# vishal-2000/EDMP

Hardware: AMD Instinct MI355X
Metric: guided denoise-steps/sec (trajectories x reverse steps) (higher is better)
Workload: dtype f32

## Files before the change

### edmp_amd/_capi.py

```python
from __future__ import annotations

import ctypes as C
import os

_HERE = os.path.dirname(os.path.abspath(__file__))
LIB_PATH = os.path.join(_HERE, "libedmp_hip.so")

MAX_LEVELS = 8
MAX_SCENES = 16
MAX_OBSTACLES = 64
MAX_SPHERES = 128
MAX_SWEEP_SUBSTEPS = 64
MAX_REPAIR_ITERS = 1024


class UNetDesc(C.Structure):
    _fields_ = [
        ("input_dim", C.c_int32),
        ("time_dim", C.c_int32),
        ("n_levels", C.c_int32),
        ("dims", C.c_int32 * MAX_LEVELS),
        ("horizon", C.c_int32),
        ("T", C.c_int32),
    ]
# ... 77 lines not shown
    "edmp_unet_flops_direct": (_i, [_vp, _pd]),
    "edmp_unet_flops_pipes": (_i, [_vp, _pd, _pd]),
    "edmp_prof_ops_bf16": (_i, [_vp, _i, C.POINTER(C.c_int), _pd]),
    "edmp_unet_slot": (_i, [_vp, C.c_uint64]),
    "edmp_guide_slot": (_i, [_vp, C.c_uint64]),
    "edmp_argmin_dev": (_i, [_vp, _vp, _i, C.POINTER(C.c_int)]),
    "edmp_sdf_set": (_i, [_vp, _pf, _i, _pi32, _pd, _pd, _i, _i]),
    "edmp_sdf_set_self": (_i, [_vp, _pi32, _pd, _pd, _i, _i]),
    "edmp_sdf_self_rows_dev": (_i, [_vp, _vp, _i, _i, _i, _i, _i, _vp, _vp]),
    "edmp_sdf_set_goal": (_i, [_vp, _pd, _pd, _pi32, _pd, _pd, _i]),
    "edmp_sdf_goal_rows_dev": (_i, [_vp, _vp, _i, _i, _i, _i, _i, _vp, _vp, _vp, _vp]),
    "edmp_sdf_set_sweep": (_i, [_vp, _pd, _pi32, _i]),
    "edmp_sdf_sweep_rows_dev": (_i, [_vp, _vp, _i, _i, _i, _pd, _pd, _i, _vp, _vp]),
    "edmp_scenes_sdf_sweep_rows_dev": (_i, [_vp, _vp, _i, _i, _i, _i, _pd, _pd, _i, _vp, _vp]),
    "edmp_sdf_repair_rows_dev": (_i, [_vp, _vp, _i, _i, _pd, _pd, _pi32, _i, _i, _i, _d, _d, _d, _d, _vp, _vp, _vp]),
    "edmp_scenes_sdf_repair_rows_dev": (_i, [_vp, _vp, _i, _i, _i, _pd, _pd, _pi32, _i, _i, _i, _d, _d, _d, _d, _vp, _vp, _vp]),
    "edmp_sdf_rows_dev": (_i, [_vp, _vp, _i, _i, _i, _pd, _pd, _vp, _vp]),
    "edmp_scene_batch_set_sdf": (_i, [_vp, _pf, _i, _pi32, _pd, _pd, _i, _i, _i]),
    "edmp_scenes_sdf_rows_dev": (_i, [_vp, _vp, _i, _i, _i, _i, _pd, _pd, _vp, _vp]),
    "edmp_sampler_set_allreduce": (_i, [_vp, _vp, _vp]),
    "edmp_rccl_load": (_i, [C.c_char_p]),
    "edmp_rccl_unique_id": (_i, [_vp]),
    "edmp_rccl_attach": (_i, [_vp, _vp, _i, _i]),
    "edmp_rccl_attach_comm": (_i, [_vp, _vp]),
    "edmp_rccl_enable": (_i, [_vp, _i]),
    "edmp_rccl_detach": (_i, [_vp]),
    "edmp_rccl_info": (_i, [_vp, _pi32]),
    "edmp_sampler_allreduce_stats": (_i, [_vp, C.POINTER(C.c_uint64), _i]),
    "edmp_prof_enable": (_i, [_vp, _i]),
    "edmp_prof_read": (_i, [_vp, _pd, C.POINTER(C.c_int64), _i]),
    "edmp_prof_ops": (_i, [_vp, _i, C.POINTER(C.c_int), _pd, C.POINTER(C.c_int64), _pd, C.c_char_p]),
    "edmp_unet_op_attrs": (_i, [_vp, _i, C.POINTER(C.c_int), C.c_char_p, _pi32, _pi32, _pi32, _pi32]),
    "edmp_cu_claim": (_i, [_i, _i, _i, _i]),
}

_lib = None


def load():
    global _lib
    if _lib is not None:
        return _lib
    if not os.path.exists(LIB_PATH):
        raise EdmpError(
            f"{LIB_PATH} is missing: build it with `python -c 'import __graft_entry__ as g; g.build()'` "
            "(hipcc --offload-arch=gfx950).  edmp_amd has no CPU fallback."
        )
    try:
        import torch
    except ImportError:
        pass
    try:
        lib = C.CDLL(LIB_PATH)
    except OSError as e:
        raise EdmpError(f"cannot load {LIB_PATH}: {e}") from e
    for name, (res, args) in SIGNATURES.items():
        try:
            fn = getattr(lib, name)
        except AttributeError as e:
            raise EdmpError(f"{LIB_PATH} does not export {name}") from e
        fn.restype = res
        fn.argtypes = args
    _lib = lib
    return lib


def check(rc: int, what: str = ""):
    if rc != 0:
        msg = load().edmp_last_error()
        err = (EdmpLayoutError if rc == ERR_LAYOUT else EdmpError)(f"{what or 'libedmp_hip'} failed (rc={rc}): {msg.decode() if msg else '?'}")
        err.rc = rc
        raise err


def as_pd(a):
    return a.ctypes.data_as(_pd)


def as_pf(a):
    return a.ctypes.data_as(_pf)


def as_pi32(a):
    return a.ctypes.data_as(_pi32)


def plan_describe(input_dim, time_dim, dims, horizon, T):
    lib = load()
    d = UNetDesc()
    d.input_dim, d.time_dim, d.n_levels, d.horizon, d.T = input_dim, time_dim, len(dims), horizon, T
    for i, v in enumerate(dims):
        d.dims[i] = v
    n, layout, size = C.c_int(), C.c_int(), C.c_int64()
    check(lib.edmp_unet_plan_describe(C.byref(d), 0, C.byref(n), None, None, None), "edmp_unet_plan_describe")
    names = C.create_string_buffer(max(n.value, 1) * 64)
    check(lib.edmp_unet_plan_describe(C.byref(d), n.value, C.byref(n), names, C.byref(layout), C.byref(size)), "edmp_unet_plan_describe")
    return [names.raw[i * 64:(i + 1) * 64].split(b"\0", 1)[0].decode() for i in range(n.value)], layout.value, size.value
```

### edmp_amd/csrc/bf3.hip

```cpp
#pragma once
#include <type_traits>

#include "params.h"
#include "wide.hip"

namespace edmp {

constexpr int kBf3Threads = 512;

typedef __attribute__((ext_vector_type(8))) __bf16 bf16x8_t;
typedef __attribute__((ext_vector_type(2))) __bf16 bf16x2_t;
typedef __attribute__((ext_vector_type(4))) float f32x4_t;
typedef __attribute__((ext_vector_type(4))) unsigned u32x4_t;
typedef __attribute__((ext_vector_type(2))) unsigned u32x2_t;

inline unsigned short bf16_rne_bits(float x) {
    unsigned u = __builtin_bit_cast(unsigned, x);
    u += 0x7fffu + ((u >> 16) & 1u);
    return (unsigned short)(u >> 16);
}
inline float bf16_bits_to_float(unsigned short b) { return __builtin_bit_cast(float, (unsigned)b << 16); }
inline void split3_bf16_rne(float x, unsigned short (&c)[3]) {
    c[0] = bf16_rne_bits(x);
    const float r1 = x - bf16_bits_to_float(c[0]);
    c[1] = bf16_rne_bits(r1);
    const float r2 = r1 - bf16_bits_to_float(c[1]);
    c[2] = bf16_rne_bits(r2);
}

template <int KIND, int MS, int CG, int GS, int LIN, bool RES>
struct Bf3Cfg {
    static constexpr int kKind = KIND, kMs = MS, kCg = CG, kGs = GS, kLin = LIN;
    static constexpr bool kRes = RES;
    static constexpr int NTH = kBf3Threads, NMW = 4;
    static constexpr int LOUT = (KIND == WK_K5) ? LIN : (KIND == WK_DOWN) ? (LIN - 1) / 2 + 1 : ((2 * LIN == 8 || 2 * LIN == 14 || 2 * LIN == 26) ? 2 * LIN - 1 : 2 * LIN);
    static constexpr bool GN = (KIND == WK_K5);
    static constexpr bool PAIRABLE = !GN && MS == 32 && CG == 32;
    using Paired = std::conditional_t<PAIRABLE, Bf3Cfg<KIND, MS, 2 * CG, 2 * CG, LIN, RES>, Bf3Cfg>;
    static constexpr int SW = 16, S = CG / SW, PARTS = NMW / S;
    static constexpr bool ROWSPLIT = (PARTS == 2 && MS == 32);
    static constexpr int NR = (PARTS == 1) ? MS / 16 : 1;
    static constexpr bool RES_ONE_ACC = RES && MS == 16 && LIN >= 13;
    static constexpr int KC = 32;
    static constexpr int RS = KC + 8;
    static constexpr int PLANE = MS * RS;
    static constexpr int STAGE = LIN * 3 * PLANE;
    static constexpr int NTAP = (KIND == WK_K5) ? 5 : (KIND == WK_DOWN) ? 3 : 4;
    static constexpr int NSLOT = NTAP + (RES ? 1 : 0);
    static constexpr int WBLK = NSLOT * 3 * 1024;
    static constexpr int slot(int l, int lp) {
        const int t = (KIND == WK_K5) ? lp - l + 2 : (KIND == WK_DOWN) ? lp - 2 * l + 1 : l + 1 - 2 * lp;
        return (t >= 0 && t < NTAP) ? t : -1;
    }
    static constexpr int NTILE = LOUT + (RES ? LIN : 0);
    static constexpr int tslot(int tile, int lp) { return tile < LOUT ? slot(tile, lp) : (tile - LOUT == lp ? NTAP : -1); }
    static constexpr int pairs_of(int l) {
        int n = (RES && l < LIN) ? 1 : 0;
        for (int lp = 0; lp < LIN; ++lp) n += slot(l, lp) >= 0 ? 1 : 0;
        return n;
    }
    static constexpr int total_pairs() {
        int n = 0;
        for (int l = 0; l < LOUT; ++l) n += pairs_of(l);
        return n;
    }
    static constexpr unsigned part0_mask() {
        if (ROWSPLIT || PARTS == 1) return ~0u;
        const int tot = total_pairs();
        int pc[16] = {};
        for (int l = 0; l < LOUT; ++l) pc[l] = pairs_of(l);
        unsigned best = 0;
// ... 5 lines not shown
            if (mx < bestmax) bestmax = mx, best = m;
        }
        return best;
    }
    static constexpr unsigned P0 = part0_mask();
    static constexpr bool owned(int tile, int H) {
        if (ROWSPLIT || PARTS == 1) return true;
        const int l = tile < LOUT ? tile : tile - LOUT;
        return (int)((P0 >> l) & 1u) == (H == 0 ? 1 : 0);
    }
    static constexpr int local(int tile, int H) {
        int n = 0;
        for (int q = 0; q < tile; ++q) n += owned(q, H) ? 1 : 0;
        return n;
    }
    static constexpr int ntiles(int H) { return local(NTILE, H); }
    static constexpr int MAXT = ntiles(0) > ntiles(1) ? ntiles(0) : ntiles(1);
    static constexpr bool needed(int H, int lp) {
        for (int t = 0; t < NTILE; ++t)
            if (owned(t, H) && tslot(t, lp) >= 0) return true;
        return false;
    }
    static constexpr int ord(int H, int q) {
        int n = 0;
        for (int i = 0; i < q; ++i) n += needed(H, i % LIN) ? 1 : 0;
        return n;
    }
    static constexpr int next(int H, int q) {
        for (int i = q + 1; i < 2 * LIN; ++i)
            if (needed(H, i % LIN)) return i;
        return -1;
    }
    static constexpr int first(int H) { return needed(H, 0) ? 0 : next(H, 0); }
    static constexpr bool DEALT = !(KIND == WK_DOWN && MS == 32);
    static constexpr int DEAL = 1;
    static constexpr int nfeed(int H, int lp, int upto = NTILE) {
        int n = 0;
        for (int t = 0; t < upto; ++t) n += (owned(t, H) && tslot(t, lp) >= 0) ? 1 : 0;
        return n;
    }
    static constexpr int nslots(int H, int q) { return DEALT ? 3 * nfeed(H, q % LIN) * NR / DEAL : 0; }
    static constexpr int nreads(int H, int q) {
        const int qn = next(H, q);
        return qn < 0 ? 0 : NR * (qn / LIN == 0 ? 2 : 3);
    }
    static constexpr int reads_dealt(int H, int q) {
        const int qn = next(H, q);
        if (qn < 0 || (ROTATE && next(H, qn) < 0)) return 0;
        return nreads(H, q) < nslots(H, q) ? nreads(H, q) : nslots(H, q);
    }
    static constexpr int nweights(int ph) { return !DEALT ? 0 : ph == 0 ? NSLOT : 2 * NSLOT; }
    static constexpr int wbase(int H, int ph, int lp) {
        int n = 0;
        for (int i = 0; i < lp; ++i)
            if (needed(H, i)) {
                const int cap = nslots(H, ph * LIN + i) - reads_dealt(H, ph * LIN + i);
                n += cap < nweights(ph) - n ? cap : nweights(ph) - n;
            }
        return n;
    }
    static constexpr int wdealt(int H, int q) { return wbase(H, q / LIN, q % LIN + 1) - wbase(H, q / LIN, q % LIN); }
    static constexpr int KREGS = MAXT * NR * 8 + 3 * NSLOT * 4 + 2 * NR * 3 * 4;
    static constexpr bool ROTATE = KREGS <= 240, BIAS_EARLY = ROTATE;
    static_assert(DEALT || ROTATE, "the burst form of the K loop is kept for rotated instances only");
    static constexpr int A_F4 = LIN * MS * (KC / 4);
    static constexpr int NA = (A_F4 + 255) / 256;
    static constexpr int YS = LOUT * CG + 4, RYS = LIN * CG + 4;
    static constexpr int PPR = NTH / MS, ROW_F4 = LOUT * CG / 4, NF4 = (ROW_F4 + PPR - 1) / PPR;
    static constexpr int RROW_F4 = LIN * CG / 4, RNF4 = (RROW_F4 + PPR - 1) / PPR;
    static constexpr size_t lds_bytes() {
        const size_t a = 2 * (size_t)STAGE * 2, y = (size_t)MS * (YS + (RES ? RYS : 0)) * 4;
        return a > y ? a : y;
    }
    static_assert((CG == 32 && S == 2 && PARTS == 2) || (CG == 64 && S == 4 && PARTS == 1 && MS == 32), "two 16-channel slabs x two parts, or four slabs = the four MFMA waves");
    static_assert(MS == 32 || MS == 16, "32 samples (sample-half parts) or 16 samples (position-set parts)");
    static_assert(!RES || KIND == WK_K5, "the folded residual 1x1 conv belongs to a Conv1dBlock");
    static_assert(!GN || CG % GS == 0, "whole GroupNorm groups per workgroup");
    static_assert((4 * PPR) % CG == 0, "a thread's columns of the final pass lie in one GroupNorm group");
    static_assert(LOUT <= 16, "part0_mask searches 2^LOUT subsets");
};

#ifdef EDMP_BF3_STAMPS
__device__ long long g_bf3_stamps[8][8];
#define EDMP_BF3_STAMP(i) \
    if (blockIdx.x == 0 && lane == 0) g_bf3_stamps[wave][i] = clock64();
#define EDMP_BF3_CHUNK_BARRIER \
    bar_t0 = clock64();        \
    __syncthreads();           \
    bar_t1 = clock64();
#define EDMP_BF3_BAR_ADD bar_cyc += bar_t1 - bar_t0;
#else
#define EDMP_BF3_STAMP(i)
#define EDMP_BF3_CHUNK_BARRIER __syncthreads();
#define EDMP_BF3_BAR_ADD
#endif

template <class Cf, class Claim>
__device__ __forceinline__ void bf3_conv_body(const float* a_src1, const float* a_src2, const void* a_W, int a_C1, int a_C2, int a_Cout, int a_B, int a_gx_shift, int a_ng_shift, const RcbP& p, Claim claim) {
    constexpr int KIND = Cf::kKind, MS = Cf::kMs, CG = Cf::kCg, GS = Cf::kGs, LIN = Cf::kLin;
    constexpr bool RES = Cf::kRes;
    constexpr int LOUT = Cf::LOUT, KC = Cf::KC, RS = Cf::RS, PLANE = Cf::PLANE, STAGE = Cf::STAGE, NSLOT = Cf::NSLOT, NTILE = Cf::NTILE, MAXT = Cf::MAXT;
    constexpr int YS = Cf::YS, RYS = Cf::RYS, NA = Cf::NA, A_F4 = Cf::A_F4, WBLK = Cf::WBLK;
    constexpr bool GN = Cf::GN;
    extern __shared__ __attribute__((aligned(16))) unsigned char lds_raw[];
    unsigned short* stg = reinterpret_cast<unsigned short*>(lds_raw);
    const int tid = threadIdx.x;
    const int lane = tid & 63;
// ... 324 lines not shown
            if (b < a_B) {
#pragma unroll
                for (int i = 0; i < NF4; ++i) {
                    const int f = epart + PPR * i;
                    if ((ROW_F4 % PPR == 0) || f < ROW_F4) {
                        const int col = 4 * f;
                        const int l = col / CG, ch = co0 + col % CG;
                        const float s0 = rstd * g4[i].x, s1 = rstd * g4[i].y, s2 = rstd * g4[i].z, s3 = rstd * g4[i].w;
                        const f32x2_t sa = {s0, s1}, sb = {s2, s3};
                        const f32x2_t ya = mish_fast2(f32x2_t{v[i].x, v[i].y} * sa + (f32x2_t{be4[i].x, be4[i].y} - sa * mean)) + f32x2_t{ad4[i].x, ad4[i].y};
                        const f32x2_t yb = mish_fast2(f32x2_t{v[i].z, v[i].w} * sb + (f32x2_t{be4[i].z, be4[i].w} - sb * mean)) + f32x2_t{ad4[i].z, ad4[i].w};
                        float4 o;
                        o.x = ya.x, o.y = ya.y, o.z = yb.x, o.w = yb.y;
                        *reinterpret_cast<float4*>(p.dst + ((size_t)b * LOUT + l) * a_Cout + ch) = o;
                    }
                }
            }
        } else if (b < a_B) {
#pragma unroll
            for (int i = 0; i < NF4; ++i) {
                const int f = epart + PPR * i;
                if ((ROW_F4 % PPR == 0) || f < ROW_F4) {
                    const int col = 4 * f;
                    const int l = col / CG, ch = co0 + col % CG;
                    *reinterpret_cast<float4*>(p.dst + ((size_t)b * LOUT + l) * a_Cout + ch) = v[i];
                }
            }
        }
    }
    EDMP_BF3_STAMP(4)
}

constexpr int kBf3PairBit = 1 << 8;

template <int KIND, int MS, int CG, int GS, int LIN, bool RES>
__global__ __launch_bounds__(kBf3Threads) void bf3_conv_kernel(const float* a_src1, const float* a_src2, const void* a_W, int a_C1, int a_C2, int a_Cout, int a_B,
                                                       int a_gx_shift, int a_ng_shift, RcbP p) {
    using Cf = Bf3Cfg<KIND, MS, CG, GS, LIN, RES>;
    const auto claim = [] __device__() __attribute__((always_inline)) {
        asm volatile("v_mov_b32 v255, 0" ::: "v255");
    };
    if constexpr (Cf::PAIRABLE) {
        const int ng_shift = a_ng_shift & (kBf3PairBit - 1);
        if (a_ng_shift & kBf3PairBit) bf3_conv_body<typename Cf::Paired>(a_src1, a_src2, a_W, a_C1, a_C2, a_Cout, a_B, a_gx_shift, ng_shift, p, claim);
        else bf3_conv_body<Cf>(a_src1, a_src2, a_W, a_C1, a_C2, a_Cout, a_B, a_gx_shift, ng_shift, p, claim);
    } else {
        bf3_conv_body<Cf>(a_src1, a_src2, a_W, a_C1, a_C2, a_Cout, a_B, a_gx_shift, a_ng_shift, p, claim);
    }
}

inline size_t bf3_stream_elems(int cout, int cin, int nslot) { return (size_t)(cout / 16) * (cin / 32) * nslot * 3 * 512; }
inline void pack_fragments_bf3(const float* w_tco_ci, int cout, int cin, int ntap, bool res, unsigned short* out) {
    const size_t n = (size_t)cout * cin;
    const int nkg = cin / 32, nslot = ntap + (res ? 1 : 0);
    for (int sl = 0; sl < cout / 16; ++sl)
        for (int kg = 0; kg < nkg; ++kg)
            for (int slot = 0; slot < nslot; ++slot) {
                const int tap = slot < ntap ? slot : 5;
                for (int lane = 0; lane < 64; ++lane) {
                    const int nn = lane % 16, oct = lane / 16;
                    for (int j = 0; j < 8; ++j) {
                        const float wv = w_tco_ci[(size_t)tap * n + (size_t)(sl * 16 + nn) * cin + 32 * kg + 8 * oct + j];
                        unsigned short c3[3];
                        split3_bf16_rne(wv, c3);
                        for (int comp = 0; comp < 3; ++comp) out[((((size_t)sl * nkg + kg) * nslot + slot) * 3 + comp) * 512 + lane * 8 + j] = c3[comp];
                    }
                }
            }
}

inline int bf3_cu_count(int* out) {
    static std::atomic<int> n_cu{0};
    int n = n_cu.load(std::memory_order_acquire);
    if (!n) {
        int dev = 0;
        EDMP_HIP_CHECK(hipGetDevice(&dev));
        EDMP_HIP_CHECK(hipDeviceGetAttribute(&n, hipDeviceAttributeMultiprocessorCount, dev));
        n_cu.store(n, std::memory_order_release);
    }
    *out = n;
    return EDMP_OK;
}

template <int KIND, int MS, int CG, int GS, int LIN, bool RES>
int launch_bf3_t(const RcbP& p, hipStream_t s, KernelAttrs* q) {
    using Cf = Bf3Cfg<KIND, MS, CG, GS, LIN, RES>;
    using Pf = typename Cf::Paired;
    static std::atomic<int> attr_set{0};
    constexpr size_t max_bytes = Cf::lds_bytes() > Pf::lds_bytes() ? Cf::lds_bytes() : Pf::lds_bytes();
    static_assert(max_bytes <= 160 * 1024, "bf16x3 position-tile kernel exceeds the 160 KiB LDS of a CU");
    size_t bytes = max_bytes;
    const void* fn = reinterpret_cast<const void*>(&bf3_conv_kernel<KIND, MS, CG, GS, LIN, RES>);
    if (!attr_set.load(std::memory_order_acquire)) {
        EDMP_HIP_CHECK(hipFuncSetAttribute(fn, hipFuncAttributeMaxDynamicSharedMemorySize, (int)bytes));
        attr_set.store(1, std::memory_order_release);
    }
    if (q) {
        hipFuncAttributes fa{};
        EDMP_HIP_CHECK(hipFuncGetAttributes(&fa, fn));
        int wg = 0;
        EDMP_HIP_CHECK(hipOccupancyMaxActiveBlocksPerMultiprocessor(&wg, fn, kBf3Threads, bytes));
        q->regs = fa.numRegs;
        q->block = kBf3Threads;
        q->lds = (int)bytes;
        q->wg_per_cu = wg;
        return EDMP_OK;
    }
    EDMP_REQUIRE(p.C1 % Cf::KC == 0 && p.C2 % Cf::KC == 0 && p.Cout % CG == 0, "bf3_conv_kernel: channels must be multiples of 32 (C1=%d, C2=%d, Cout=%d)", p.C1, p.C2, p.Cout);
    EDMP_REQUIRE(p.C2 == 0 || p.C2 == p.C1, "bf3_conv_kernel: the two halves of a concatenated input must have the same width (C1=%d, C2=%d)", p.C1, p.C2);
    int ng = p.Cout / CG;
    const int nt = (p.B + MS - 1) / MS;
    bool pair = false;
    if constexpr (Cf::PAIRABLE) {
        int n_cu = 0;
        if (const int rc = bf3_cu_count(&n_cu); rc != EDMP_OK) return rc;
        pair = ng % 2 == 0 && ng * nt > n_cu;
    }
    if (pair) {
        EDMP_REQUIRE(p.Cout % Pf::kCg == 0, "bf3_conv_kernel: paired workgroups need Cout to be a multiple of %d (Cout=%d)", Pf::kCg, p.Cout);
        ng = p.Cout / Pf::kCg;
    }
    bytes = pair ? Pf::lds_bytes() : Cf::lds_bytes();
    const int gx = xcd_split(ng, nt, (double)p.Cout * (p.C1 + p.C2) * Cf::NSLOT * 1.5, (double)nt * MS * LIN * (p.C1 + p.C2));
    int gxs = -1, ngs = -1;
    if (gx > 0 && (ng & (ng - 1)) == 0) {
        gxs = __builtin_ctz(gx);
        ngs = __builtin_ctz(ng);
    }
    if constexpr (Cf::PAIRABLE) ngs = (ngs < 0 ? 0 : ngs) | (pair ? kBf3PairBit : 0);
    hipLaunchKernelGGL((bf3_conv_kernel<KIND, MS, CG, GS, LIN, RES>), dim3(ng * nt), dim3(kBf3Threads), bytes, s, p.src1, p.src2, reinterpret_cast<const void*>(p.W), p.C1, p.C2, p.Cout, p.B, gxs, ngs, p);
    return EDMP_OK;
}

}
```

### edmp_amd/csrc/params.h

```cpp
#pragma once
#include "common.h"
#include "tail.h"

namespace edmp {

struct ConvP {
    const float* src1;
    const float* src2;
    int C1, C2;
    int Lin, Lout;
    int ntaps, stride, pad, transposed;
    const float* W;
    const float* bias;
    float* dst;
    int Cout;
    int B;
};

struct GnP {
    float* y;
    const float* gamma;
    const float* beta;
    const float* add_res;
    const float* add_tbias;
    int L, C, B;
};

struct RcbP {
    const float* src1;
    const float* src2;
    int C1, C2;
    const float* W;
    const float* bias;
    const float* gamma;
    const float* beta;
    const float* add_tb;
    const float* add_res;
    float* dst;
    int Cout;
    int B;
    float* res_out;
    const float* res_bias;
    int gx_shift = -1, ng_shift = -1;
};

struct KernelAttrs {
    int regs = 0;
    int block = 0;
    int lds = 0;
    int wg_per_cu = 0;
};

enum LevelMode { LV_DOWN = 0, LV_UP = 1, LV_UP_FINAL = 2 };

struct LevelP {
    const float* src1;
    const float* src2;
    int C1, C2;
    const float* w11;
    const float* w12;
    const float* w21;
    const float* w22;
    const float* wrs;
    const float* wfin;
    const float *b11, *g11, *be11, *tb1, *rb1;
    const float *b12, *g12, *be12;
    const float *b21, *g21, *be21, *tb2;
    const float *b22, *g22, *be22;
    const float* brs;
    const float *bfin, *gfin, *befin;
    float* skip_out;
    float* out;
    int B;
    TailP tail;
};

#ifdef EDMP_STAMPS
#ifdef EDMP_STAMPS_DEFINE
__device__ unsigned long long g_stamps[8][16];
#else
extern __device__ unsigned long long g_stamps[8][16];
#endif
#define EDMP_STAMP(k, i)                                                        \
// ... 24 lines not shown
```

### edmp_amd/csrc/unet.hip

```cpp
#include <memory>
#include <variant>

#include "common.h"
#define EDMP_STAMPS_DEFINE 1
#include "params.h"

namespace edmp {

using f32x16 = __attribute__((ext_vector_type(16))) float;

struct RawT {
    int64_t off;
    int d0, d1, d2;
};
struct RawConvBlock {
    RawT w, b, gw, gb;
};
struct RawRCB {
    RawConvBlock cb[2];
    RawT tw, tb;
    bool has_res;
    RawT rw, rb;
    int cin, cout;
};
// ... 506 lines not shown
    const bool wide = (p.Cout % 64 == 0);
    if (wide) {
        if (kc == 64) launch_conv_t<64, 64, 64>(p, s);
        else if (kc == 32) launch_conv_t<64, 64, 32>(p, s);
        else if (kc == 16) launch_conv_t<64, 64, 16>(p, s);
        else launch_conv_t<64, 64, 8>(p, s);
    } else {
        if (kc >= 32) launch_conv_t<128, 32, 32>(p, s);
        else if (kc == 16) launch_conv_t<128, 32, 16>(p, s);
        else launch_conv_t<128, 32, 8>(p, s);
    }
}
static int launch_gn(const GnP& p, hipStream_t s) {
    const int n = (p.C / 8) * p.L;
    dim3 grid((p.B * 8 + 3) / 4);
    if (n <= 128) hipLaunchKernelGGL((gn_mish_kernel<2>), grid, dim3(256), 0, s, p);
    else if (n <= 256) hipLaunchKernelGGL((gn_mish_kernel<4>), grid, dim3(256), 0, s, p);
    else if (n <= 512) hipLaunchKernelGGL((gn_mish_kernel<8>), grid, dim3(256), 0, s, p);
    else {
        set_error("GroupNorm group of %d elements exceeds the register-resident limit (512)", n);
        return EDMP_ERR_ARG;
    }
    return EDMP_OK;
}

static const int kBf3Default = 0xff;
static const int kMs16Default = 0x05;
static const char kLevelSbDefault[] = "4222";
static const int kLevelMergeDefault = 0x3;
struct BuildSwitches {
    bool fused, resfold, level, karatsuba;
    int bf3, ms16, level_merge;
    int level_sb[4];
    static BuildSwitches read() {
        auto env = [](const char* name) { return getenv(name); };
        auto mask = [&](const char* name, int dflt) { const char* e = env(name); return e ? (int)strtol(e, nullptr, 0) : dflt; };
        BuildSwitches s;
        s.fused = env("EDMP_NO_FUSED") == nullptr;
        s.resfold = env("EDMP_NO_RESFOLD") == nullptr;
        s.level = s.fused && env("EDMP_NO_LEVEL") == nullptr;
        s.karatsuba = env("EDMP_NO_KARATSUBA") == nullptr;
        s.bf3 = mask("EDMP_BF16X3", kBf3Default);
        s.ms16 = mask("EDMP_MS16", kMs16Default);
        s.level_merge = mask("EDMP_LEVEL_MERGE", kLevelMergeDefault);
        const char* e = env("EDMP_LEVEL_SB");
        for (int d = 0; d < 4; ++d) s.level_sb[d] = ((e && strlen(e) == 4) ? e : kLevelSbDefault)[d] == '2' ? 2 : 4;
        return s;
    }
};

enum PackForm : uint64_t { F_CONV = 1, F_CONVT = 2, F_FRAG = 3, F_FRAG_K2 = 4, F_FRAG_K4 = 5, F_RESAMPLE = 6, F_VEC = 7, F_FRAG_BF3 = 8 };

static const struct { int kind, cg, L, bf3_bit, ms16_bit; } kConvFamilies[] = {
    {WK_K5, 32, 7, 0, 0},    {WK_K5, 16, 7, 1, -1},   {WK_K5, 16, 13, 2, -1},
    {WK_K5, 64, 4, 6, -1},   {WK_K5, 32, 4, 7, -1},
    {WK_DOWN, 32, 7, 3, 1},  {WK_UP, 32, 4, 3, 2},
    {WK_DOWN, 64, 4, 4, 3},  {WK_UP, 64, 2, 4, 4},
    {WK_DOWN, 16, 13, 5, -1}, {WK_UP, 16, 7, 5, -1},
};

struct ConvChoice {
    const ConvInst* row[2] = {nullptr, nullptr};
    int form = 0;
    PackForm stream = F_FRAG;
};
static ConvChoice choose_conv(const BuildSwitches& sw, int kind, int cout, int L, int c1, int c2) {
    ConvChoice c;
    if (!sw.fused || cout % 8 != 0 || c1 % 32 != 0 || c2 % 32 != 0 || (c2 != 0 && c2 != c1)) return c;
    const int cg = cout / 8;
    int bf3_bit = -1, ms16_bit = -1;
    for (const auto& f : kConvFamilies)
        if (f.kind == kind && f.cg == cg && f.L == L) bf3_bit = f.bf3_bit, ms16_bit = f.ms16_bit;
    const bool bf3 = bf3_bit >= 0 && (sw.bf3 >> bf3_bit & 1);
    int ms, cgw = std::max(cg, 32), gs = cg;
    if (bf3) {
        ms = cg >= 32 ? 32 : 16;
        if (kind != WK_K5) cgw = 32, gs = std::min(cg, 32);
// ... 275 lines not shown
    static long valid_pairs(int Lin, int Lout, int k, int stride, int pad, bool tr) {
        long cnt = 0;
        for (int lo = 0; lo < Lout; ++lo)
            for (int t = 0; t < k; ++t) {
                if (!tr) {
                    int li = lo * stride + t - pad;
                    if (li >= 0 && li < Lin) ++cnt;
                } else {
                    int num = lo + pad - t;
                    if (num >= 0 && num % stride == 0 && num / stride < Lin) ++cnt;
                }
            }
        return cnt;
    }
    static void conv_flops(Op& o, int Lin, int Lout, int cin_true, int cin_store, int Cout, int k, int stride, int pad, bool tr) {
        o.flops_nominal = tr ? 2.0 * Lin * cin_true * Cout * k : 2.0 * Lout * Cout * (double)cin_true * k;
        o.flops_exec = 2.0 * (double)valid_pairs(Lin, Lout, k, stride, pad, tr) * Cout * (double)cin_store;
    }
    TH emit_conv(TH a, const TH* a2, int cin_true, size_t w, size_t b, int Cout, int k, int stride, int pad, bool tr, int Lout) {
        ConvP c{};
        set_src(c, a, a2);
        c.Lin = a.L, c.Lout = Lout, c.ntaps = k, c.stride = stride, c.pad = pad, c.transposed = tr;
        c.W = bind.w(w), c.bias = bind.w(b), c.Cout = Cout;
        const TH out = new_out(Cout, a.L, Lout);
        c.dst = bind.buf(out.buf);
        Op o{OP_CONV, c};
        conv_flops(o, a.L, Lout, cin_true, c.C1 + c.C2, Cout, k, stride, pad, tr);
        push(o);
        return out;
    }
    TH emit_wrs(TH a, size_t w, size_t b, int Cout, const ConvInst* inst, int k, int Lout) {
        RcbP c{};
        set_src(c, a, nullptr);
        c.W = bind.w(w), c.bias = bind.w(b), c.Cout = Cout;
        const TH out = new_out(Cout, a.L, Lout);
        c.dst = bind.buf(out.buf);
        Op o{OP_WRS, c};
        o.inst = inst;
        conv_flops(o, a.L, Lout, a.C, a.C, Cout, k, 2, 1, inst->kind == WK_UP);
        push(o);
        return out;
    }
    void emit_gn(TH y, const float* gamma, const float* beta, const float* res, int tb_off) {
        GnP g{};
        g.y = bind.buf(y.buf), g.gamma = gamma, g.beta = beta, g.add_res = res, g.L = y.L, g.C = y.C;
        if (!gn_group && (y.C / 8) * y.L > 512) gn_group = (y.C / 8) * y.L;
        Op o{OP_GN, g};
        o.tb1 = tb_off;
        push(o);
    }
    TH emit_resampler(int kind, TH a, const RawT& w, const RawT& b, int Lout) {
        const bool up = kind == WK_UP;
        const int C = a.C, k = up ? 4 : 3;
        if (const ConvChoice ch = choose_conv(sw, kind, C, a.L, C, 0); ch.row[0]) {
            const size_t wo = pk.resample_frag(params + w.off, C, C, k, up, ch.stream, ch.row[0]->ms), bo = pk.vec(params + b.off, C);
            return emit_wrs(a, wo, bo, C, ch.row[0], k, Lout);
        }
        const size_t wo = up ? pk.convT(params + w.off, C, C, k) : pk.conv(params + w.off, C, C, k, C), bo = pk.vec(params + b.off, C);
        return emit_conv(a, nullptr, C, wo, bo, C, k, 2, 1, up, Lout);
    }
    TH emit_res_conv(const RawRCB& r, TH x, const TH* x2) {
        const size_t wr = pk.conv(params + r.rw.off, r.cout, r.cin, 1, x.C + (x2 ? x2->C : 0)), br = pk.vec(params + r.rb.off, r.cout);
        return emit_conv(x, x2, r.cin, wr, br, r.cout, 1, 1, 0, false, x.L);
    }
    struct BlockW { const float *w, *b, *gamma, *beta; };
    TH emit_fused(TH a, const TH* a2, int cin_true, int cout, const ConvChoice& ch, const BlockW& w, const float* res, int tbo, const RawT* fold_bias, TH* fold) {
        RcbP c{};
        set_src(c, a, a2);
        c.W = w.w, c.bias = w.b, c.gamma = w.gamma, c.beta = w.beta, c.add_res = res, c.Cout = cout;
        const TH out = new_out(cout, a.L, a.L);
        c.dst = bind.buf(out.buf);
        const int cin_store = c.C1 + c.C2;
        Op o{OP_RCB};
        o.tb1 = tbo;
        o.inst = ch.row[fold ? 1 : 0];
        if (!o.inst && !no_twin_cout) no_twin_cout = cout, no_twin_L = a.L;
        conv_flops(o, a.L, a.L, cin_true, cin_store, cout, 5, 1, 2, false);
        o.flops_direct = o.flops_exec;
        if (ch.form) o.flops_exec = 2.0 * (ch.form == 2 ? 3.0 : 9.0) * cout * (double)cin_store;
        if (fold) {
            *fold = TH{pool.get(), cout, a.L};
            c.res_out = bind.buf(fold->buf);
            c.res_bias = vec(*fold_bias, cout);
            o.flops_nominal += 2.0 * a.L * cout * (double)cin_true;
            o.flops_exec += 2.0 * a.L * cout * (double)cin_store;
            o.flops_direct += 2.0 * a.L * cout * (double)cin_store;
        }
        o.p = c;
        push(o);
        return out;
    }
    TH emit_rcb(TH x, const TH* x2) {
        const RawRCB& r = inv.rcbs[rcb_idx++];
        const int cin_store = x.C + (x2 ? x2->C : 0);
        const ConvChoice ch1 = choose_conv(sw, WK_K5, r.cout, x.L, x.C, x2 ? x2->C : 0), ch2 = choose_conv(sw, WK_K5, r.cout, x.L, r.cout, 0);
        const bool wide = ch1.row[0] && ch2.row[0];
        const bool fold_res = wide && r.has_res && sw.resfold;
        const size_t w1 = wide ? pk.conv_frag(params + r.cb[0].w.off, fold_res ? params + r.rw.off : nullptr, r.cout, r.cin, cin_store, x.L, ch1.stream, ch1.row[0]->ms)
                               : pk.conv(params + r.cb[0].w.off, r.cout, r.cin, 5, cin_store);
        const size_t b1 = pk.vec(params + r.cb[0].b.off, r.cout);
        const BlockW k1{bind.w(w1), bind.w(b1), vec(r.cb[0].gw, r.cout), vec(r.cb[0].gb, r.cout)};
        const size_t w2 = wide ? pk.conv_frag(params + r.cb[1].w.off, nullptr, r.cout, r.cout, r.cout, x.L, ch2.stream, ch2.row[0]->ms) : pk.conv(params + r.cb[1].w.off, r.cout, r.cout, 5, r.cout);
// ... 478 lines not shown
}

extern "C" int edmp_prof_ops_bf16(edmp_ctx* ctx, int cap, int* n_ops, double* flops_bf16) {
    EDMP_REQUIRE(ctx && ctx->unet && n_ops, "edmp_prof_ops_bf16: null argument / no model");
    const int n = (int)ctx->unet->prog.size();
    *n_ops = n;
    for (int i = 0; i < n && i < cap; ++i)
        if (flops_bf16) flops_bf16[i] = ctx->unet->prog[i].flops_bf16;
    return EDMP_OK;
}

extern "C" int edmp_prof_ops(edmp_ctx* ctx, int cap, int* n_ops, double* ms, int64_t* calls, double* flops_exec, char* names) {
    EDMP_REQUIRE(ctx && ctx->unet && n_ops, "edmp_prof_ops: null argument / no model");
    EDMP_HIP_CHECK(hipSetDevice(ctx->device));
    EDMP_HIP_CHECK(hipStreamSynchronize(ctx->stream));
    if (int rc = prof_fold(ctx)) return rc;
    const int n = (int)ctx->unet->prog.size();
    *n_ops = n;
    for (int i = 0; i < n && i < cap; ++i) {
        const Op& op = ctx->unet->prog[i];
        if (ms) ms[i] = ctx->prof.op_ms[i];
        if (calls) calls[i] = ctx->prof.op_calls[i];
        if (flops_exec) flops_exec[i] = op.flops_exec;
        if (names) {
            strncpy(names + (size_t)i * 64, op.name, 63);
            names[(size_t)i * 64 + 63] = 0;
        }
    }
    return EDMP_OK;
}

extern "C" int edmp_cu_claim(int regs, int block, int lds_bytes, int wg_per_cu) { return owns_cu(regs, block, lds_bytes, wg_per_cu) ? 1 : 0; }

extern "C" int edmp_unet_op_attrs(edmp_ctx* ctx, int cap, int* n_ops, char* names, int* regs, int* block, int* lds_bytes, int* wg_per_cu) {
    EDMP_REQUIRE(ctx && ctx->unet && n_ops, "edmp_unet_op_attrs: null argument / no model");
    const int n = (int)ctx->unet->prog.size();
    *n_ops = n;
    for (int i = 0; i < n && i < cap; ++i) {
        const Op& op = ctx->unet->prog[i];
        if (names) {
            strncpy(names + (size_t)i * 64, op.name, 63);
            names[(size_t)i * 64 + 63] = 0;
        }
        if (regs) regs[i] = op.attrs.regs;
        if (block) block[i] = op.attrs.block;
        if (lds_bytes) lds_bytes[i] = op.attrs.lds;
        if (wg_per_cu) wg_per_cu[i] = op.attrs.wg_per_cu;
    }
    return EDMP_OK;
}

#ifdef EDMP_STAMPS
extern "C" int edmp_debug_stamps(unsigned long long* out) {
    return (int)hipMemcpyFromSymbol(out, HIP_SYMBOL(edmp::g_stamps), sizeof(unsigned long long) * 8 * 16);
}
#endif
```

### include/edmp_hip.h

```cpp
#ifndef EDMP_HIP_H
#define EDMP_HIP_H

#include <stddef.h>
#include <stdint.h>

#ifdef __cplusplus
extern "C" {
#endif

#define EDMP_OK 0
#define EDMP_ERR_ARG (-1)
#define EDMP_ERR_HIP (-2)
#define EDMP_ERR_STATE (-3)
#define EDMP_ERR_LAYOUT (-4)

#define EDMP_MAX_LEVELS 8
#define EDMP_N_JOINTS 7
#define EDMP_N_LINKS 9
#define EDMP_MAX_OBSTACLES 64
#define EDMP_MAX_SCENES 16
#define EDMP_MAX_SPHERES 128
#define EDMP_MAX_SWEEP_SUBSTEPS 64
#define EDMP_MAX_REPAIR_ITERS 1024

// ... 140 lines not shown
int edmp_denoise_scenes_rng_segment_dev(edmp_ctx* ctx, const uint64_t* seeds, int S, int B, const double* starts, const double* goals, int guided,
                                        int t_hi, int t_lo, int init, int zero_row0, double* X_out_dev);
int edmp_sampler_seed_rng_dev(edmp_ctx* ctx, const double* x0_dev, int x0_rows, uint64_t seed, int renoise, int B, const double* start,
                              const double* goal, int guided, int t_start, double* X_out_dev);
int edmp_sampler_seed_scenes_rng_dev(edmp_ctx* ctx, const double* x0_dev, int x0_rows, const uint64_t* seeds, int renoise, int S, int B,
                                     const double* starts, const double* goals, int guided, int t_start, double* X_out_dev);

int edmp_sampler_set_graph(edmp_ctx* ctx, int on);

int edmp_q_sample_dev(edmp_ctx* ctx, const double* x_dev, const double* eps_dev, const int32_t* t_host, int B, int C, int N,
                      int cumulative, int condition, double* xt_dev, double* mean_dev);

int edmp_unet_slot(edmp_ctx* ctx, uint64_t key);
int edmp_guide_slot(edmp_ctx* ctx, uint64_t key);

typedef int (*edmp_allreduce_fn)(void* user, void* hip_stream, double* sumsq_dev);
int edmp_sampler_set_allreduce(edmp_ctx* ctx, edmp_allreduce_fn fn, void* user);

int edmp_rccl_load(const char* path);
int edmp_rccl_unique_id(void* id128);
int edmp_rccl_attach(edmp_ctx* ctx, const void* id128, int nranks, int rank);
int edmp_rccl_attach_comm(edmp_ctx* ctx, void* nccl_comm);
int edmp_rccl_enable(edmp_ctx* ctx, int on);
int edmp_rccl_detach(edmp_ctx* ctx);
int edmp_rccl_info(edmp_ctx* ctx, int32_t out[3]);
int edmp_sampler_allreduce_stats(edmp_ctx* ctx, uint64_t out[3], int reset);

int edmp_prof_enable(edmp_ctx* ctx, int on);
int edmp_prof_read(edmp_ctx* ctx, double* conv_ms, int64_t* conv_launches, int reset);
int edmp_prof_ops(edmp_ctx* ctx, int cap, int* n_ops, double* ms, int64_t* calls, double* flops_exec, char* names);
int edmp_prof_ops_bf16(edmp_ctx* ctx, int cap, int* n_ops, double* flops_bf16);
int edmp_unet_op_attrs(edmp_ctx* ctx, int cap, int* n_ops, char* names, int* regs, int* block, int* lds_bytes, int* wg_per_cu);
int edmp_cu_claim(int regs, int block, int lds_bytes, int wg_per_cu);

#ifdef __cplusplus
}
#endif
#endif
```

Baseline: 1.208 million.

## Add half-tile bf16x3 conv workgroup organisation with 16 samples and 64 channels

Adds a Half configuration for eligible bf16x3 conv instances: each workgroup covers 16 samples by 64 output channels instead of 32 by 32, selected at launch when it yields at least as many workgroups, or when forced through EDMP_BF3_HALF. Launch organisation is factored into a shared helper and exposed through a query API. The aim is to reshape tiles so weight reuse across channels rises while the grid keeps enough workgroups, but each instance now compiles an extra body variant, which may raise code size and register pressure.

Result: no change. 1.214 million, median of 6 (+0.5%).

```diff
diff --git a/edmp_amd/_capi.py b/edmp_amd/_capi.py
--- a/edmp_amd/_capi.py
+++ b/edmp_amd/_capi.py
@@ -133,6 +133,7 @@
     "edmp_prof_ops": (_i, [_vp, _i, C.POINTER(C.c_int), _pd, C.POINTER(C.c_int64), _pd, C.c_char_p]),
     "edmp_unet_op_attrs": (_i, [_vp, _i, C.POINTER(C.c_int), C.c_char_p, _pi32, _pi32, _pi32, _pi32]),
     "edmp_cu_claim": (_i, [_i, _i, _i, _i]),
+    "edmp_bf3_launch_org": (_i, [_i] * 10 + [_pi32, _pi32, _pi32]),
 }
 
 _lib = None
@@ -197,3 +198,13 @@
     names = C.create_string_buffer(max(n.value, 1) * 64)
     check(lib.edmp_unet_plan_describe(C.byref(d), n.value, C.byref(n), names, C.byref(layout), C.byref(size)), "edmp_unet_plan_describe")
     return [names.raw[i * 64:(i + 1) * 64].split(b"\0", 1)[0].decode() for i in range(n.value)], layout.value, size.value
+
+
+BF3_ORGS = ("listed", "paired", "half")
+
+
+def bf3_launch_org(inst, cout, B, cus, half_tiles=0):
+    kind, ms, cg, gs, L, res = inst
+    org, wgs, lds = C.c_int32(), C.c_int32(), C.c_int32()
+    check(load().edmp_bf3_launch_org(kind, ms, cg, gs, L, int(res), cout, B, half_tiles, cus, C.byref(org), C.byref(wgs), C.byref(lds)), "edmp_bf3_launch_org")
+    return BF3_ORGS[org.value], wgs.value, lds.value
diff --git a/edmp_amd/csrc/bf3.hip b/edmp_amd/csrc/bf3.hip
--- a/edmp_amd/csrc/bf3.hip
+++ b/edmp_amd/csrc/bf3.hip
@@ -37,6 +37,8 @@
     static constexpr bool GN = (KIND == WK_K5);
     static constexpr bool PAIRABLE = !GN && MS == 32 && CG == 32;
     using Paired = std::conditional_t<PAIRABLE, Bf3Cfg<KIND, MS, 2 * CG, 2 * CG, LIN, RES>, Bf3Cfg>;
+    static constexpr bool HALVABLE = MS == 32 && CG == 32 && GS == 32 && ((KIND == WK_K5 && !(LIN == 7 && RES)) || (KIND == WK_DOWN && LIN == 7) || (KIND == WK_UP && LIN == 4));
+    using Half = std::conditional_t<HALVABLE, Bf3Cfg<KIND, MS / 2, 2 * CG, GS, LIN, RES>, Bf3Cfg>;
     static constexpr int SW = 16, S = CG / SW, PARTS = NMW / S;
     static constexpr bool ROWSPLIT = (PARTS == 2 && MS == 32);
     static constexpr int NR = (PARTS == 1) ? MS / 16 : 1;
@@ -108,7 +110,7 @@
         return -1;
     }
     static constexpr int first(int H) { return needed(H, 0) ? 0 : next(H, 0); }
-    static constexpr bool DEALT = !(KIND == WK_DOWN && MS == 32);
+    static constexpr bool DEALT = !(KIND == WK_DOWN && (MS == 32 || CG == 64));
     static constexpr int DEAL = 1;
     static constexpr int nfeed(int H, int lp, int upto = NTILE) {
         int n = 0;
@@ -148,7 +150,7 @@
         const size_t a = 2 * (size_t)STAGE * 2, y = (size_t)MS * (YS + (RES ? RYS : 0)) * 4;
         return a > y ? a : y;
     }
-    static_assert((CG == 32 && S == 2 && PARTS == 2) || (CG == 64 && S == 4 && PARTS == 1 && MS == 32), "two 16-channel slabs x two parts, or four slabs = the four MFMA waves");
+    static_assert((CG == 32 && S == 2 && PARTS == 2) || (CG == 64 && S == 4 && PARTS == 1 && NR == MS / 16), "two 16-channel slabs x two parts, or four slabs = the four MFMA waves (two row blocks each, or one: Half)");
     static_assert(MS == 32 || MS == 16, "32 samples (sample-half parts) or 16 samples (position-set parts)");
     static_assert(!RES || KIND == WK_K5, "the folded residual 1x1 conv belongs to a Conv1dBlock");
     static_assert(!GN || CG % GS == 0, "whole GroupNorm groups per workgroup");
@@ -539,6 +541,7 @@
 }
 
 constexpr int kBf3PairBit = 1 << 8;
+constexpr int kBf3HalfBit = 1 << 9;
 
 template <int KIND, int MS, int CG, int GS, int LIN, bool RES>
 __global__ __launch_bounds__(kBf3Threads) void bf3_conv_kernel(const float* a_src1, const float* a_src2, const void* a_W, int a_C1, int a_C2, int a_Cout, int a_B,
@@ -547,9 +550,10 @@
     const auto claim = [] __device__() __attribute__((always_inline)) {
         asm volatile("v_mov_b32 v255, 0" ::: "v255");
     };
-    if constexpr (Cf::PAIRABLE) {
+    if constexpr (Cf::PAIRABLE || Cf::HALVABLE) {
         const int ng_shift = a_ng_shift & (kBf3PairBit - 1);
-        if (a_ng_shift & kBf3PairBit) bf3_conv_body<typename Cf::Paired>(a_src1, a_src2, a_W, a_C1, a_C2, a_Cout, a_B, a_gx_shift, ng_shift, p, claim);
+        if (Cf::PAIRABLE && (a_ng_shift & kBf3PairBit)) bf3_conv_body<typename Cf::Paired>(a_src1, a_src2, a_W, a_C1, a_C2, a_Cout, a_B, a_gx_shift, ng_shift, p, claim);
+        else if (Cf::HALVABLE && (a_ng_shift & kBf3HalfBit)) bf3_conv_body<typename Cf::Half>(a_src1, a_src2, a_W, a_C1, a_C2, a_Cout, a_B, a_gx_shift, ng_shift, p, claim);
         else bf3_conv_body<Cf>(a_src1, a_src2, a_W, a_C1, a_C2, a_Cout, a_B, a_gx_shift, ng_shift, p, claim);
     } else {
         bf3_conv_body<Cf>(a_src1, a_src2, a_W, a_C1, a_C2, a_Cout, a_B, a_gx_shift, a_ng_shift, p, claim);
@@ -589,10 +593,35 @@
     return EDMP_OK;
 }
 
+enum Bf3Org { BF3_LISTED = 0, BF3_PAIRED = 1, BF3_HALF = 2 };
+struct Bf3Launch {
+    int org, ng, nt, ms;
+    size_t lds;
+};
+template <class Cf>
+inline Bf3Launch bf3_organise(const RcbP& p, int n_cu) {
+    using Pf = typename Cf::Paired;
+    using Hf = typename Cf::Half;
+    static_assert(Hf::lds_bytes() <= Cf::lds_bytes(), "a half-tile workgroup stages and hands over no more than the listed one");
+    const int ng = p.Cout / Cf::kCg, nt = (p.B + Cf::kMs - 1) / Cf::kMs;
+    if (Cf::PAIRABLE && ng % 2 == 0 && ng * nt > n_cu) return {BF3_PAIRED, p.Cout / Pf::kCg, nt, Pf::kMs, Pf::lds_bytes()};
+    if (Cf::HALVABLE && ng % 2 == 0 && p.half_tiles >= 0) {
+        const int nth = (p.B + Hf::kMs - 1) / Hf::kMs;
+        if (p.half_tiles > 0 || nth * (ng / 2) >= nt * ng) return {BF3_HALF, p.Cout / Hf::kCg, nth, Hf::kMs, Hf::lds_bytes()};
+    }
+    return {BF3_LISTED, ng, nt, Cf::kMs, Cf::lds_bytes()};
+}
+
 template <int KIND, int MS, int CG, int GS, int LIN, bool RES>
 int launch_bf3_t(const RcbP& p, hipStream_t s, KernelAttrs* q) {
     using Cf = Bf3Cfg<KIND, MS, CG, GS, LIN, RES>;
     using Pf = typename Cf::Paired;
+    if (q && q->cus > 0) {
+        EDMP_REQUIRE(p.B > 0 && p.Cout > 0 && p.Cout % CG == 0, "bf3_conv_kernel: cannot organise a launch of B=%d, Cout=%d", p.B, p.Cout);
+        const Bf3Launch o = bf3_organise<Cf>(p, q->cus);
+        q->org = o.org, q->grid = o.ng * o.nt, q->block = kBf3Threads, q->lds = (int)o.lds;
+        return EDMP_OK;
+    }
     static std::atomic<int> attr_set{0};
     constexpr size_t max_bytes = Cf::lds_bytes() > Pf::lds_bytes() ? Cf::lds_bytes() : Pf::lds_bytes();
     static_assert(max_bytes <= 160 * 1024, "bf16x3 position-tile kernel exceeds the 160 KiB LDS of a CU");
@@ -615,26 +644,20 @@
     }
     EDMP_REQUIRE(p.C1 % Cf::KC == 0 && p.C2 % Cf::KC == 0 && p.Cout % CG == 0, "bf3_conv_kernel: channels must be multiples of 32 (C1=%d, C2=%d, Cout=%d)", p.C1, p.C2, p.Cout);
     EDMP_REQUIRE(p.C2 == 0 || p.C2 == p.C1, "bf3_conv_kernel: the two halves of a concatenated input must have the same width (C1=%d, C2=%d)", p.C1, p.C2);
-    int ng = p.Cout / CG;
-    const int nt = (p.B + MS - 1) / MS;
-    bool pair = false;
+    int n_cu = 0;
     if constexpr (Cf::PAIRABLE) {
-        int n_cu = 0;
         if (const int rc = bf3_cu_count(&n_cu); rc != EDMP_OK) return rc;
-        pair = ng % 2 == 0 && ng * nt > n_cu;
-    }
-    if (pair) {
-        EDMP_REQUIRE(p.Cout % Pf::kCg == 0, "bf3_conv_kernel: paired workgroups need Cout to be a multiple of %d (Cout=%d)", Pf::kCg, p.Cout);
-        ng = p.Cout / Pf::kCg;
-    }
-    bytes = pair ? Pf::lds_bytes() : Cf::lds_bytes();
-    const int gx = xcd_split(ng, nt, (double)p.Cout * (p.C1 + p.C2) * Cf::NSLOT * 1.5, (double)nt * MS * LIN * (p.C1 + p.C2));
+    }
+    const Bf3Launch o = bf3_organise<Cf>(p, n_cu);
+    const int ng = o.ng, nt = o.nt;
+    bytes = o.lds;
+    const int gx = xcd_split(ng, nt, (double)p.Cout * (p.C1 + p.C2) * Cf::NSLOT * 1.5, (double)nt * o.ms * LIN * (p.C1 + p.C2));
     int gxs = -1, ngs = -1;
     if (gx > 0 && (ng & (ng - 1)) == 0) {
         gxs = __builtin_ctz(gx);
         ngs = __builtin_ctz(ng);
     }
-    if constexpr (Cf::PAIRABLE) ngs = (ngs < 0 ? 0 : ngs) | (pair ? kBf3PairBit : 0);
+    if constexpr (Cf::PAIRABLE || Cf::HALVABLE) ngs = (ngs < 0 ? 0 : ngs) | (o.org == BF3_PAIRED ? kBf3PairBit : o.org == BF3_HALF ? kBf3HalfBit : 0);
     hipLaunchKernelGGL((bf3_conv_kernel<KIND, MS, CG, GS, LIN, RES>), dim3(ng * nt), dim3(kBf3Threads), bytes, s, p.src1, p.src2, reinterpret_cast<const void*>(p.W), p.C1, p.C2, p.Cout, p.B, gxs, ngs, p);
     return EDMP_OK;
 }
diff --git a/edmp_amd/csrc/params.h b/edmp_amd/csrc/params.h
--- a/edmp_amd/csrc/params.h
+++ b/edmp_amd/csrc/params.h
@@ -42,6 +42,7 @@
     float* res_out;
     const float* res_bias;
     int gx_shift = -1, ng_shift = -1;
+    int half_tiles = 0;
 };
 
 struct KernelAttrs {
@@ -49,6 +50,7 @@
     int block = 0;
     int lds = 0;
     int wg_per_cu = 0;
+    int cus = 0, org = 0, grid = 0;
 };
 
 enum LevelMode { LV_DOWN = 0, LV_UP = 1, LV_UP_FINAL = 2 };
diff --git a/edmp_amd/csrc/unet.hip b/edmp_amd/csrc/unet.hip
--- a/edmp_amd/csrc/unet.hip
+++ b/edmp_amd/csrc/unet.hip
@@ -562,6 +562,7 @@
     bool fused, resfold, level, karatsuba;
     int bf3, ms16, level_merge;
     int level_sb[4];
+    int half_tiles;
     static BuildSwitches read() {
         auto env = [](const char* name) { return getenv(name); };
         auto mask = [&](const char* name, int dflt) { const char* e = env(name); return e ? (int)strtol(e, nullptr, 0) : dflt; };
@@ -573,6 +574,8 @@
         s.bf3 = mask("EDMP_BF16X3", kBf3Default);
         s.ms16 = mask("EDMP_MS16", kMs16Default);
         s.level_merge = mask("EDMP_LEVEL_MERGE", kLevelMergeDefault);
+        const char* h = env("EDMP_BF3_HALF");
+        s.half_tiles = !h ? 0 : (!strcmp(h, "on") || !strcmp(h, "1")) ? 1 : (!strcmp(h, "off") || !strcmp(h, "0")) ? -1 : 0;
         const char* e = env("EDMP_LEVEL_SB");
         for (int d = 0; d < 4; ++d) s.level_sb[d] = ((e && strlen(e) == 4) ? e : kLevelSbDefault)[d] == '2' ? 2 : 4;
         return s;
@@ -914,7 +917,7 @@
     TH emit_wrs(TH a, size_t w, size_t b, int Cout, const ConvInst* inst, int k, int Lout) {
         RcbP c{};
         set_src(c, a, nullptr);
-        c.W = bind.w(w), c.bias = bind.w(b), c.Cout = Cout;
+        c.W = bind.w(w), c.bias = bind.w(b), c.Cout = Cout, c.half_tiles = sw.half_tiles;
         const TH out = new_out(Cout, a.L, Lout);
         c.dst = bind.buf(out.buf);
         Op o{OP_WRS, c};
@@ -949,7 +952,7 @@
     TH emit_fused(TH a, const TH* a2, int cin_true, int cout, const ConvChoice& ch, const BlockW& w, const float* res, int tbo, const RawT* fold_bias, TH* fold) {
         RcbP c{};
         set_src(c, a, a2);
-        c.W = w.w, c.bias = w.b, c.gamma = w.gamma, c.beta = w.beta, c.add_res = res, c.Cout = cout;
+        c.W = w.w, c.bias = w.b, c.gamma = w.gamma, c.beta = w.beta, c.add_res = res, c.Cout = cout, c.half_tiles = sw.half_tiles;
         const TH out = new_out(cout, a.L, a.L);
         c.dst = bind.buf(out.buf);
         const int cin_store = c.C1 + c.C2;
@@ -1494,6 +1497,20 @@
 
 extern "C" int edmp_cu_claim(int regs, int block, int lds_bytes, int wg_per_cu) { return owns_cu(regs, block, lds_bytes, wg_per_cu) ? 1 : 0; }
 
+extern "C" int edmp_bf3_launch_org(int kind, int ms, int cg, int gs, int L, int res, int cout, int B, int half_tiles, int cus, int* org, int* workgroups, int* lds_bytes) {
+    EDMP_REQUIRE(org && workgroups && cus > 0, "edmp_bf3_launch_org: null argument / no CU count");
+    const ConvInst* inst = find_conv(true, kind, ms, cg, gs, L, res != 0);
+    EDMP_REQUIRE(inst, "edmp_bf3_launch_org: no instance bf3_conv_kernel<%d, %d, %d, %d, %d, %s>", kind, ms, cg, gs, L, res ? "true" : "false");
+    RcbP p{};
+    p.Cout = cout, p.B = B, p.half_tiles = half_tiles;
+    KernelAttrs a;
+    a.cus = cus;
+    if (int rc = inst->launch(p, nullptr, &a)) return rc;
+    *org = a.org, *workgroups = a.grid;
+    if (lds_bytes) *lds_bytes = a.lds;
+    return EDMP_OK;
+}
+
 extern "C" int edmp_unet_op_attrs(edmp_ctx* ctx, int cap, int* n_ops, char* names, int* regs, int* block, int* lds_bytes, int* wg_per_cu) {
     EDMP_REQUIRE(ctx && ctx->unet && n_ops, "edmp_unet_op_attrs: null argument / no model");
     const int n = (int)ctx->unet->prog.size();
diff --git a/include/edmp_hip.h b/include/edmp_hip.h
--- a/include/edmp_hip.h
+++ b/include/edmp_hip.h
@@ -196,6 +196,7 @@
 int edmp_prof_ops_bf16(edmp_ctx* ctx, int cap, int* n_ops, double* flops_bf16);
 int edmp_unet_op_attrs(edmp_ctx* ctx, int cap, int* n_ops, char* names, int* regs, int* block, int* lds_bytes, int* wg_per_cu);
 int edmp_cu_claim(int regs, int block, int lds_bytes, int wg_per_cu);
+int edmp_bf3_launch_org(int kind, int ms, int cg, int gs, int L, int res, int cout, int B, int half_tiles, int cus, int* org, int* workgroups, int* lds_bytes);
 
 #ifdef __cplusplus
 }
```
